# Hi-FT/ERD

Measured on AMD Instinct MI355X. Metric: images/sec GFL-R50 40+40 incre step @1333x800, higher is better.
Workload: dtype f32; 1 GPU; gfl_r50_fpn first_40_incre_last_40 ERD (BASELINE configs[1]), 1333x800 padded to 800x1344, fp32, procedural weights; batch_per_gpu=4, global_batch=4, parallelism=dp1

## Files before the change

### erd_amd/csrc/conv_mfma.hip

```cpp
#include <algorithm>
#include <type_traits>
#include "erd_common.h"
#include <stdlib.h>
#ifndef ERD_SGB
#define ERD_SGB 0
#endif

namespace {

typedef float f32x16 __attribute__((ext_vector_type(16)));
typedef __bf16 bf16x8 __attribute__((ext_vector_type(8)));
typedef __bf16 bf16x2v __attribute__((ext_vector_type(2)));
typedef float f32x2v __attribute__((ext_vector_type(2)));

__device__ __forceinline__ float pack_bf16(float a, float b) {
    const f32x2v v = {a, b};
    return __builtin_bit_cast(float, __builtin_convertvector(v, bf16x2v));
}

constexpr int NTHREADS = 256;

#ifdef ERD_IGEMM_TRACE
__device__ unsigned long long g_igemm_trace[1024 * 8];
#define IG_T0(v) const unsigned long long v = __builtin_amdgcn_s_memtime()
#define IG_ACC(slot, v) if (threadIdx.x == 0 && blockIdx.x < 1024) g_igemm_trace[blockIdx.x * 8 + slot] += __builtin_amdgcn_s_memtime() - v
#define IG_SET(slot, val) if (threadIdx.x == 0 && blockIdx.x < 1024) g_igemm_trace[blockIdx.x * 8 + slot] = (val)
#else
#define IG_T0(v)
#define IG_ACC(slot, v)
#define IG_SET(slot, val)
#endif

struct RowInfo {
    int in_off;
    int ih0, iw0;
    int out_off;
};

__device__ __forceinline__ int swz(int row, int chunk) { return chunk ^ ((row >> 1) & 7); }

typedef unsigned int u32x4 __attribute__((ext_vector_type(4)));
constexpr unsigned OOB = 0x7fffffffu;

__device__ __forceinline__ float4 buf_load16(__amdgpu_buffer_rsrc_t r, unsigned byte_off) {
    const u32x4 v = __builtin_amdgcn_raw_buffer_load_b128(r, byte_off, 0, 0);
    return make_float4(__uint_as_float(v.x), __uint_as_float(v.y), __uint_as_float(v.z), __uint_as_float(v.w));
}

typedef int i32x4 __attribute__((ext_vector_type(4)));
__device__ __forceinline__ i32x4 rsrc_words(const void* ptr, int bytes) {
    const unsigned long long a = (unsigned long long)ptr;
    i32x4 r;
    r.x = __builtin_amdgcn_readfirstlane((int)(unsigned)a);
    r.y = __builtin_amdgcn_readfirstlane((int)((a >> 32) & 0xffffu));
    r.z = __builtin_amdgcn_readfirstlane(bytes);
    r.w = 0x00020000;
    return r;
}
__device__ __forceinline__ void glds16(const i32x4 rs, unsigned lds_byte, unsigned voff) {
    asm volatile("s_mov_b32 m0, %0\n\ts_nop 0\n\tbuffer_load_dwordx4 %1, %2, 0 offen lds" ::"s"(lds_byte), "v"(voff), "s"(rs) : "memory");
}
__device__ __forceinline__ void glds_wait_all() { asm volatile("s_waitcnt vmcnt(0)" ::: "memory"); }

struct SkWs {
    int* cnt;
    float* slabs;
    int xcd_order;
    int whole_tiles;
};

int xcd_order_enabled() {
    static const int v = getenv("ERD_XCD") ? atoi(getenv("ERD_XCD")) : 1;
    return v;
}

template <int BM, int BN, int WAVES_M, int WAVES_N, int BKT, int MINW, bool BF = false, bool ST = false, bool AB = false,
          bool OB = false, bool X3 = false, bool RES = false, bool MSK = false,
          bool GL = false>
__global__ __launch_bounds__(WAVES_M * WAVES_N * 64, MINW) void conv_igemm_kernel(const erd_conv_desc p, const int total_tiles,
                                                                     const SkWs ws) {
    constexpr int NT = WAVES_M * WAVES_N * 64;
    constexpr int FM = BM / (WAVES_M * 32);
    constexpr int FN = BN / (WAVES_N * 32);
    constexpr int CH = BKT / 4;
    constexpr int RPP = NT / CH;
    constexpr int AJ = BM / RPP;
    constexpr int BJ = BN / RPP;
    constexpr int KPC = BF ? 8 : 4;
    constexpr int BK = CH * KPC;
    constexpr bool SGB = ERD_SGB;
    static_assert(WAVES_M * WAVES_N == 4 || (WAVES_M * WAVES_N == 8 && BF && !X3), "4 waves (8: bf16 matrix cores only)");
    static_assert(BF || (!AB && !OB), "bf16 storage only with the bf16 matrix cores");
    static_assert(!X3 || (!BF && BKT == 32 && WAVES_N == 1 && FM == 1), "f32x3: fp32 maps, 32-channel slices, 4 x 1 waves");
    static_assert(!GL || X3, "LDS-DMA staging: the three-limb kernel (both operands are stored in LDS exactly as they lie in memory)");
    constexpr unsigned ABYTES = AB ? 2u : 4u;
    constexpr int CHB = X3 ? 4 : CH;
    constexpr int NPL = X3 ? 3 : 1;
    constexpr int RPPB = NT / CHB;
    constexpr int BJX = BN / RPPB;

    extern __shared__ __attribute__((aligned(16))) char smem[];
    float4* As = reinterpret_cast<float4*>(smem);
    float4* Bs = As + 2 * BM * CH;
    constexpr int OPER_BYTES = 2 * (BM * CH + NPL * BN * CHB) * 16;
    constexpr int STAGE_BYTES = 64 * (BN + 4) * 4 + NT * 16;
    constexpr int REGION = OPER_BYTES > STAGE_BYTES ? OPER_BYTES : STAGE_BYTES;
    constexpr int WSTAGE_BYTES = 32 * (BN + 4) * 4;
    constexpr int ROWS_EPI_OFF = X3 ? ((4 * WSTAGE_BYTES + 255) / 256 * 256) : REGION;
    static_assert(!X3 || ROWS_EPI_OFF + BM * (int)sizeof(RowInfo) + 64 + 4 * (BN / 4) * 16 <= OPER_BYTES,
                  "f32x3: row table + column-sum scratch do not fit behind the staging blocks");
    RowInfo* rows = reinterpret_cast<RowInfo*>(smem + (X3 ? 0 : REGION));
    RowInfo* rows_epi = reinterpret_cast<RowInfo*>(smem + ROWS_EPI_OFF);
    int* bcast = reinterpret_cast<int*>(reinterpret_cast<RowInfo*>(smem + ROWS_EPI_OFF) + BM);

    const int tid = threadIdx.x;
    const int ntn = (p.Cout + BN - 1) / BN;
    const int Cin = p.Cin;
    const int cpt = (Cin + BK - 1) / BK;
    const int nkt = p.ntaps * cpt;
    const float* __restrict__ w = p.w;

    const long long U = (long long)total_tiles * nkt;
    const int G = gridDim.x;
    int wg = blockIdx.x;
    if (ws.xcd_order) {
        const int q = G >> 3, r = G & 7, xcd = blockIdx.x & 7, idx = blockIdx.x >> 3;
        wg = (xcd < r ? xcd * (q + 1) : r * (q + 1) + (xcd - r) * q) + idx;
    }
    const long long u_begin = ws.whole_tiles ? ((long long)total_tiles * wg / G) * nkt : (U * wg) / G;
    const long long u_end = ws.whole_tiles ? ((long long)total_tiles * (wg + 1) / G) * nkt : (U * (wg + 1)) / G;

    const int chunk = tid % CH;
    const int r0 = tid / CH;
    auto swzc = [](int row, int c) { return CH == 8 ? (c ^ ((row >> 1) & 7)) : (c ^ ((row >> 2) & 3)); };
    const int wave = tid >> 6, lane = tid & 63;
    const int chunk_l = GL ? (chunk ^ ((r0 >> 1) & 7)) : chunk;
    const int wave_s = __builtin_amdgcn_readfirstlane(wave);
    const int wm = wave / WAVES_N, wn = wave % WAVES_N;
    const int li = lane & 31, h = lane >> 5;

    IG_T0(t_kernel);
    IG_SET(0, t_kernel);
    for (int q_ = 1; q_ < 8; ++q_) { IG_SET(q_, 0ull); }
    for (long long u = u_begin; u < u_end;) {
        IG_T0(t_pro);
        const int tt = (int)(u / nkt);
        const int ks = (int)(u - (long long)tt * nkt);
        int ke = (int)min((long long)nkt, ks + (u_end - u));
        u += ke - ks;
        const int nt = tt % ntn;
        int mt = tt / ntn;

        int s = 0;
#pragma unroll 1
        for (; s < p.nseg - 1; ++s) {
            const int M = p.seg[s].N * p.seg[s].GH * p.seg[s].GW;
            const int tiles = (M + BM - 1) / BM;
            if (mt < tiles) break;
            mt -= tiles;
        }
        const erd_conv_seg& sg = p.seg[s];
        const int IH = sg.IH, IW = sg.IW;
        const float* __restrict__ in = sg.in;
        const int tap_lo = (ST && sg.ntaps) ? sg.tap0 : 0, nt_s = (ST && sg.ntaps) ? sg.ntaps : p.ntaps;
        const int oy_s = (ST && sg.ntaps) ? sg.oy : p.oy, ox_s = (ST && sg.ntaps) ? sg.ox : p.ox;
        const int nkt_t = ST ? nt_s * cpt : nkt;
        if (ST) {
            ke = min(ke, nkt_t);
            if (ks >= ke) continue;
        }

        __syncthreads();
        auto fill_rows = [&](RowInfo* dst) {
            if (tid < BM) {
                const int GHW = sg.GH * sg.GW;
                const int M = sg.N * GHW;
                const int m = mt * BM + tid;
                RowInfo ri;
                if (m < M) {
                    const int n = m / GHW;
                    const int rem = m - n * GHW;
                    const int a = rem / sg.GW;
                    const int b = rem - a * sg.GW;
                    ri.in_off = (int)(n * sg.in_nstride);
                    ri.ih0 = a * p.in_stride;
                    ri.iw0 = b * p.in_stride;
                    ri.out_off = (int)(n * sg.out_nstride) +
                                 ((a * p.out_stride + oy_s) * sg.OW + (b * p.out_stride + ox_s)) * p.Cout;
                } else {
                    ri.in_off = 0;
                    ri.ih0 = -(1 << 28);
                    ri.iw0 = -(1 << 28);
                    ri.out_off = -1;
                }
                dst[tid] = ri;
            }
        };
        if constexpr (!GL) {
            fill_rows(rows);
            __syncthreads();
        }

        unsigned a_base[AJ], a_mask[AJ];
#pragma unroll
        for (int j = 0; j < AJ; ++j) {
            RowInfo ri;
            if constexpr (GL) {
                const int GHW = sg.GH * sg.GW;
                const int m = mt * BM + r0 + RPP * j;
                if (m < sg.N * GHW) {
                    const int n = m / GHW;
                    const int rem = m - n * GHW;
                    const int a = rem / sg.GW;
                    ri.in_off = (int)(n * sg.in_nstride);
                    ri.ih0 = a * p.in_stride;
                    ri.iw0 = (rem - a * sg.GW) * p.in_stride;
                } else {
                    ri.in_off = 0;
                    ri.ih0 = -(1 << 28);
                    ri.iw0 = -(1 << 28);
                }
            } else {
                ri = rows[r0 + RPP * j];
            }
            a_base[j] = (unsigned)(ri.in_off + (ri.ih0 * IW + ri.iw0) * Cin + chunk_l * KPC) * ABYTES;
            unsigned m = 0;
            for (int t = 0; t < nt_s; ++t) {
                const int ih = ri.ih0 + p.dy[tap_lo + t], iw = ri.iw0 + p.dx[tap_lo + t];
                m |= ((unsigned)ih < (unsigned)IH && (unsigned)iw < (unsigned)IW) ? (1u << t) : 0u;
            }
            a_mask[j] = m;
        }
        const int n0 = nt * BN;
        unsigned b_base[X3 ? 1 : BJ];
        unsigned bx_base[X3 ? BJX : 1];
        const int chunkb = tid % CHB, rb0 = tid / CHB;
        const int chunkb_l = GL ? (chunkb ^ ((rb0 >> 2) & 3)) : chunkb;
        if constexpr (X3) {
#pragma unroll
            for (int j = 0; j < BJX; ++j) {
                const int co = n0 + rb0 + RPPB * j;
                bx_base[j] = co < p.Cout ? (unsigned)(co * p.wrow + chunkb_l * 8) * 2u : OOB;
            }
        } else {
#pragma unroll
            for (int j = 0; j < BJ; ++j) {
                const int co = n0 + r0 + RPP * j;
                b_base[j] = co < p.Cout ? (unsigned)(co * p.wrow + chunk * KPC) * (BF ? 2u : 4u) : OOB;
            }
        }
        const __amdgpu_buffer_rsrc_t rs_in = __builtin_amdgcn_make_buffer_rsrc(
            const_cast<float*>(in), 0, (int)((long long)sg.N * sg.in_nstride * ABYTES), 0x00020000);
        const unsigned plane_b = (unsigned)((long long)p.Cout * p.wrow * 2);
        const __amdgpu_buffer_rsrc_t rs_w = __builtin_amdgcn_make_buffer_rsrc(
            X3 ? const_cast<void*>(p.w_x3) : (BF ? const_cast<void*>(p.w_bf16) : (void*)const_cast<float*>(w)), 0,
            (int)((long long)p.Cout * p.wrow * (X3 ? 6 : (BF ? 2 : 4))), 0x00020000);
        if constexpr (X3 && !GL) __syncthreads();

        constexpr bool PD2 = BF && MINW <= 2;
        constexpr int NSET = PD2 ? 2 : 1;
        constexpr int NBL = X3 ? 3 * BJX : BJ;
        float4 ra[GL ? 1 : NSET][GL ? 1 : AJ], rb[GL ? 1 : NSET][GL ? 1 : NBL];
        float4 ra1[NSET][(BF && !AB) ? AJ : 1];
        bool cokb = false;
        int tap = ks / cpt, cc = ks - tap * cpt;
        int adelta = 0, bdelta = 0, ctap = 0;
        bool cok = false, cok1 = false;
        auto slice_begin = [&]() {
            const int cb = cc * BK;
            ctap = tap;
            adelta = ((p.dy[tap_lo + tap] * IW + p.dx[tap_lo + tap]) * Cin + cb) * (int)ABYTES;
            bdelta = (p.wk[tap_lo + tap] + cb) * ((BF || X3) ? 2 : 4);
            cok = cb + chunk_l * KPC < Cin;
            cokb = X3 && cb + chunkb_l * 8 < Cin;
            cok1 = BF && !AB && cb + chunk * KPC + 4 < Cin;
            if (++cc == cpt) { cc = 0; ++tap; }
        };
        typedef __attribute__((address_space(3))) void* lds_ptr_t;
        const unsigned lds0 = (unsigned)(size_t)(lds_ptr_t)smem;
        const i32x4 rw_in = GL ? rsrc_words(in, (int)((long long)sg.N * sg.in_nstride * ABYTES)) : i32x4{0, 0, 0, 0};
        const i32x4 rw_w = GL ? rsrc_words(p.w_x3, (int)((long long)p.Cout * p.wrow * 6)) : i32x4{0, 0, 0, 0};
        auto glds_a = [&](int j, const int buf) {
            const bool ok = cok && ((a_mask[j] >> ctap) & 1u);
            glds16(rw_in, lds0 + (unsigned)(((buf * BM + RPP * j + 8 * wave_s) * CH) * 16), ok ? a_base[j] + (unsigned)adelta : OOB);
        };
        auto glds_b = [&](int j, const int buf) {
            const int pl = j / BJX, jj = j - pl * BJX;
            glds16(rw_w, lds0 + (unsigned)((2 * BM * CH + (buf * 3 + pl) * BN * CHB + (RPPB * jj + 16 * wave_s) * CHB) * 16),
                   cokb ? bx_base[X3 ? jj : 0] + (unsigned)bdelta + (unsigned)pl * plane_b : OOB);
        };
        auto load_a = [&](int j, const int set) {
            const bool ok = cok && ((a_mask[j] >> ctap) & 1u);
            ra[set][j] = buf_load16(rs_in, ok ? a_base[j] + (unsigned)adelta : OOB);
            if (BF && !AB) ra1[set][j] = buf_load16(rs_in, (ok && cok1) ? a_base[j] + (unsigned)adelta + 16u : OOB);
        };
        auto load_b = [&](int j, const int set) {
            if constexpr (X3) {
                const int pl = j / BJX, jj = j - pl * BJX;
                rb[set][j] = buf_load16(rs_w, cokb ? bx_base[jj] + (unsigned)bdelta + (unsigned)pl * plane_b : OOB);
            } else {
                rb[set][j] = buf_load16(rs_w, cok ? b_base[X3 ? 0 : j] + (unsigned)bdelta : OOB);
            }
        };
        auto store_lds = [&](int buf, const int set) {
#pragma unroll
            for (int j = 0; j < AJ; ++j) {
                const int row = r0 + RPP * j;
                if (BF && !AB)
                    As[buf * BM * CH + row * CH + swzc(row, chunk)] =
                        make_float4(pack_bf16(ra[set][j].x, ra[set][j].y), pack_bf16(ra[set][j].z, ra[set][j].w),
                                    pack_bf16(ra1[set][(BF && !AB) ? j : 0].x, ra1[set][(BF && !AB) ? j : 0].y),
                                    pack_bf16(ra1[set][(BF && !AB) ? j : 0].z, ra1[set][(BF && !AB) ? j : 0].w));
                else
                    As[buf * BM * CH + row * CH + swzc(row, chunk)] = ra[set][j];
            }
            if constexpr (X3) {
#pragma unroll
                for (int j = 0; j < 3 * BJX; ++j) {
                    const int pl = j / BJX, row = rb0 + RPPB * (j - pl * BJX);
                    Bs[(buf * 3 + pl) * BN * CHB + row * CHB + (chunkb ^ ((row >> 2) & 3))] = rb[set][j];
                }
            } else {
#pragma unroll
                for (int j = 0; j < BJ; ++j) {
                    const int row = r0 + RPP * j;
                    Bs[buf * BN * CH + row * CH + swzc(row, chunk)] = rb[set][X3 ? 0 : j];
                }
            }
        };

        f32x16 acc[FM][FN];
#pragma unroll
        for (int i = 0; i < FM; ++i)
#pragma unroll
            for (int j = 0; j < FN; ++j)
#pragma unroll
                for (int r = 0; r < 16; ++r) acc[i][j][r] = 0.f;

        slice_begin();
        if constexpr (GL) {
#pragma unroll
            for (int j = 0; j < NBL; ++j) glds_b(j, 0);
#pragma unroll
            for (int j = 0; j < AJ; ++j) glds_a(j, 0);
        } else {
#pragma unroll
        for (int j = 0; j < AJ; ++j) load_a(j, 0);
#pragma unroll
        for (int j = 0; j < NBL; ++j) load_b(j, 0);
        }
        if (PD2 && ks + 1 < ke) {
            slice_begin();
#pragma unroll
            for (int j = 0; j < AJ; ++j) load_a(j, NSET - 1);
#pragma unroll
            for (int j = 0; j < NBL; ++j) load_b(j, NSET - 1);
        }
        if constexpr (GL) glds_wait_all(); else store_lds(0, 0);
        __syncthreads();

        IG_ACC(2, t_pro);
        IG_T0(t_loop);
        constexpr int KSTEPS = X3 ? 2 : CH / 2;
        constexpr int APS = (AJ + KSTEPS - 1) / KSTEPS, BPS = (NBL + KSTEPS - 1) / KSTEPS;
        auto k_slice_x3 = [&](const int kt, const int par) {
            const int buf = par;
            const bool more = kt + 1 < ke;
            if (more) slice_begin();
            const float4* Ab = As + buf * BM * CH;
            const float4* Bb = Bs + buf * 3 * BN * CHB;
            const int arow = wm * 32 + li;
            typedef unsigned int u4v __attribute__((ext_vector_type(4)));
            auto limb = [&](const float (&v)[8], u4v& P) {
#pragma unroll
                for (int e = 0; e < 4; ++e) P[e] = erd::pack2_bf16(v[2 * e], v[2 * e + 1]);
                return __builtin_bit_cast(bf16x8, P);
            };
            auto rest = [&](const float (&v)[8], const u4v& P, float (&r)[8]) {
#pragma unroll
                for (int e = 0; e < 4; ++e) {
                    r[2 * e] = erd::scalar_op(v[2 * e] - erd::bf16_lo(P[e]));
                    r[2 * e + 1] = erd::scalar_op(v[2 * e + 1] - erd::bf16_hi(P[e]));
                }
            };
            auto read_a = [&](int kk, float (&x)[8]) {
                const int ca = 4 * kk + 2 * h;
                const float4 x0 = Ab[arow * CH + swzc(arow, ca)], x1 = Ab[arow * CH + swzc(arow, ca + 1)];
                x[0] = x0.x; x[1] = x0.y; x[2] = x0.z; x[3] = x0.w; x[4] = x1.x; x[5] = x1.y; x[6] = x1.z; x[7] = x1.w;
            };
            float4 wb[FN][3];
            auto read_b = [&](int kk, const int pl) {
                const int cbk = 2 * kk + h;
#pragma unroll
                for (int j = 0; j < FN; ++j) {
                    const int row = j * 32 + li;
                    wb[j][pl] = Bb[pl * BN * CHB + row * CHB + (cbk ^ ((row >> 2) & 3))];
                }
            };
#ifdef ERD_X3_NOMFMA
#define ERD_X3(AV, PL)                                                                                              \
            _Pragma("unroll") for (int j = 0; j < FN; ++j) acc[0][j][PL] += wb[j][PL].x * __builtin_bit_cast(float4, AV).x;
#else
#define ERD_X3(AV, PL)                                                                                              \
            _Pragma("unroll") for (int j = 0; j < FN; ++j)                                                          \
                acc[0][j] = __builtin_amdgcn_mfma_f32_32x32x16_bf16(AV, __builtin_bit_cast(bf16x8, wb[j][PL]), acc[0][j], 0, 0, 0);
#endif
            float x[8], xn[8];
            read_a(0, x);
            read_b(0, 2);
            read_b(0, 1);
            read_b(0, 0);
#pragma unroll
            for (int kk = 0; kk < 2; ++kk) {
                if (kk == 0) read_a(1, xn);
#ifndef ERD_X3_NOLOAD
                if (more) {
#pragma unroll
                    for (int q = 0; q < APS; ++q)
                        if (kk * APS + q < AJ) { if constexpr (GL) glds_a(kk * APS + q, buf ^ 1); else load_a(kk * APS + q, 0); }
#pragma unroll
                    for (int q = 0; q < BPS; ++q)
                        if (kk * BPS + q < NBL) { if constexpr (GL) glds_b(kk * BPS + q, buf ^ 1); else load_b(kk * BPS + q, 0); }
                }
#endif
                u4v ph, pm, pl;
                const bf16x8 ah = limb(x, ph);
                ERD_X3(ah, 2)
#ifndef ERD_X3_NOBREAD
                if (kk == 0) read_b(1, 2);
#endif
                ERD_X3(ah, 1)
                ERD_X3(ah, 0)
                float r1[8], r2[8];
#ifdef ERD_X3_NOVALU
                const bf16x8 am = ah, al = ah;
                (void)r1; (void)r2;
#else
                rest(x, ph, r1);
                const bf16x8 am = limb(r1, pm);
#endif
                ERD_X3(am, 1)
#ifndef ERD_X3_NOBREAD
                if (kk == 0) read_b(1, 1);
#endif
                ERD_X3(am, 0)
#ifndef ERD_X3_NOVALU
                rest(r1, pm, r2);
                const bf16x8 al = limb(r2, pl);
#endif
                ERD_X3(al, 0)
#ifdef ERD_X3_NINE
                ERD_X3(am, 2)
                ERD_X3(al, 1)
                ERD_X3(al, 2)
#endif
                if (kk == 0) {
#ifndef ERD_X3_NOBREAD
                    read_b(1, 0);
#endif
#pragma unroll
                    for (int e = 0; e < 8; ++e) x[e] = xn[e];
                }
            }
#undef ERD_X3
#ifndef ERD_X3_NOSYNC
            if constexpr (GL) glds_wait_all(); else { if (more) store_lds(buf ^ 1, 0); }
            __syncthreads();
#endif
        };
        auto k_slice = [&](const int kt, const int par) {
            const int buf = par;
            const bool more = kt + 1 < ke;
            const bool fetch = PD2 ? kt + 2 < ke : more;
            const int fset = PD2 ? par : 0;
            if (fetch) slice_begin();
            const float4* Ab = As + buf * BM * CH;
            const float4* Bb = Bs + buf * BN * CH;
            float4 fa[2][FM], fb[2][FN];
            auto read_frags = [&](int kk, int slot) {
                const int c = 2 * kk + h;
#pragma unroll
                for (int i = 0; i < FM; ++i) {
                    const int row = (wm * FM + i) * 32 + li;
                    fa[slot][i] = Ab[row * CH + swzc(row, c)];
                }
#pragma unroll
                for (int j = 0; j < FN; ++j) {
                    const int row = (wn * FN + j) * 32 + li;
                    fb[slot][j] = Bb[row * CH + swzc(row, c)];
                }
            };
            read_frags(0, 0);
#pragma unroll
            for (int kk = 0; kk < KSTEPS; ++kk) {
                const int cur = kk & 1;
#ifndef ERD_IG_NOFRAG
                if (kk + 1 < KSTEPS) read_frags(kk + 1, cur ^ 1);
#endif
#ifdef ERD_IG_NOLOAD
                if (false) {
#else
                if (fetch) {
#endif
#pragma unroll
                    for (int q = 0; q < APS; ++q)
                        if (kk * APS + q < AJ) load_a(kk * APS + q, fset);
#pragma unroll
                    for (int q = 0; q < BPS; ++q)
                        if (kk * BPS + q < BJ) load_b(kk * BPS + q, fset);
                }
#pragma unroll
                for (int i = 0; i < FM; ++i)
#pragma unroll
                    for (int j = 0; j < FN; ++j) {
                        if (BF) {
#ifdef ERD_IG_NOMFMA
                            acc[i][j][kk] += fa[cur][i].x * fb[cur][j].y;
                            continue;
#endif
                            acc[i][j] = __builtin_amdgcn_mfma_f32_32x32x16_bf16(
                                __builtin_bit_cast(bf16x8, fa[cur][i]), __builtin_bit_cast(bf16x8, fb[cur][j]),
                                acc[i][j], 0, 0, 0);
                            continue;
                        }
                        acc[i][j] = __builtin_amdgcn_mfma_f32_32x32x2f32(fa[cur][i].x, fb[cur][j].x, acc[i][j], 0, 0, 0);
                        acc[i][j] = __builtin_amdgcn_mfma_f32_32x32x2f32(fa[cur][i].y, fb[cur][j].y, acc[i][j], 0, 0, 0);
                        acc[i][j] = __builtin_amdgcn_mfma_f32_32x32x2f32(fa[cur][i].z, fb[cur][j].z, acc[i][j], 0, 0, 0);
                        acc[i][j] = __builtin_amdgcn_mfma_f32_32x32x2f32(fa[cur][i].w, fb[cur][j].w, acc[i][j], 0, 0, 0);
                    }
                if (SGB) {
                    __builtin_amdgcn_sched_group_barrier(0x100, FM + FN, 0);
                    __builtin_amdgcn_sched_group_barrier(0x20, APS + BPS, 0);
                    __builtin_amdgcn_sched_group_barrier(0x8, FM * FN * 4, 0);
                }
            }
#ifndef ERD_IG_NOSYNC
            if (more) store_lds(buf ^ 1, PD2 ? (par ^ 1) : 0);
            __syncthreads();
#endif
        };
        if constexpr (X3) {
            for (int kt = ks; kt < ke; ++kt) k_slice_x3(kt, (kt - ks) & 1);
        } else if constexpr (PD2) {
            for (int kt = ks; kt < ke; kt += 2) {
                k_slice(kt, 0);
                if (kt + 1 < ke) k_slice(kt + 1, 1);
            }
        } else {
            for (int kt = ks; kt < ke; ++kt) k_slice(kt, (kt - ks) & 1);
        }

        IG_ACC(3, t_loop);
        IG_SET(6, g_igemm_trace[blockIdx.x * 8 + 6] + (unsigned long long)(ke - ks));
        IG_T0(t_fix);
        if (ks != 0 || ke != nkt_t) {
            const long long t0 = (long long)tt * nkt;
            const int first_b = (int)(((t0 + 1) * G - 1) / U);
            const int last_b = (int)(((t0 + nkt) * G - 1) / U);
            const int ncontrib = last_b - first_b + 1;
            const int my_slot = (tt == (int)(u_begin / nkt)) ? 0 : 1;
            const __amdgpu_buffer_rsrc_t rs_slab = __builtin_amdgcn_make_buffer_rsrc(
                ws.slabs, 0, (int)std::min<size_t>((size_t)2 * G * BM * BN * 4, 0x7fffffffu), 0x00020000);
            const unsigned slab_off = (unsigned)((size_t)(2 * wg + my_slot) * (BM * BN) * 4) + (unsigned)tid * 16u;
#pragma unroll
            for (int i = 0; i < FM; ++i)
#pragma unroll
                for (int j = 0; j < FN; ++j)
#pragma unroll
                    for (int g = 0; g < 4; ++g) {
                        u32x4 v;
                        v.x = __float_as_uint(acc[i][j][4 * g]); v.y = __float_as_uint(acc[i][j][4 * g + 1]);
                        v.z = __float_as_uint(acc[i][j][4 * g + 2]); v.w = __float_as_uint(acc[i][j][4 * g + 3]);
                        __builtin_amdgcn_raw_buffer_store_b128(v, rs_slab, slab_off + (unsigned)(((i * FN + j) * 4 + g) * NT * 16), 0, 16 );
                    }
            asm volatile("s_waitcnt vmcnt(0)" ::: "memory");
            __syncthreads();
            if (tid == 0) bcast[0] = __hip_atomic_fetch_add(ws.cnt + tt, 1, __ATOMIC_RELAXED, __HIP_MEMORY_SCOPE_AGENT);
            __syncthreads();
            if (bcast[0] != ncontrib - 1) { IG_ACC(4, t_fix); IG_SET(1, __builtin_amdgcn_s_memtime()); continue; }
            const bool pair = ncontrib == 2;
            if (!pair) {
#pragma unroll
                for (int i = 0; i < FM; ++i)
#pragma unroll
                    for (int j = 0; j < FN; ++j)
#pragma unroll
                        for (int r = 0; r < 16; ++r) acc[i][j][r] = 0.f;
            }
            for (int c = 0; c < ncontrib; ++c) {
                const int bb = first_b + c;
                if (pair && bb == wg) continue;
                const int bfirst_tile = (int)(((U * bb) / G) / nkt);
                const unsigned so = (unsigned)((size_t)(2 * bb + (tt == bfirst_tile ? 0 : 1)) * (BM * BN) * 4) + (unsigned)tid * 16u;
#pragma unroll
                for (int i = 0; i < FM; ++i)
#pragma unroll
                    for (int j = 0; j < FN; ++j)
#pragma unroll
                        for (int g = 0; g < 4; ++g) {
                            const u32x4 v = __builtin_amdgcn_raw_buffer_load_b128(
                                rs_slab, so + (unsigned)(((i * FN + j) * 4 + g) * NT * 16), 0, 16 );
                            acc[i][j][4 * g] += __uint_as_float(v.x); acc[i][j][4 * g + 1] += __uint_as_float(v.y);
                            acc[i][j][4 * g + 2] += __uint_as_float(v.z); acc[i][j][4 * g + 3] += __uint_as_float(v.w);
                        }
            }
            if (tid == 0) ws.cnt[tt] = 0;
        }

        IG_ACC(4, t_fix);
        IG_T0(t_epi);
        if constexpr (X3) fill_rows(rows_epi);
        using OutT = typename std::conditional<OB, erd::bf16s, float>::type;
        OutT* __restrict__ out = reinterpret_cast<OutT*>(sg.out);
        const OutT* res = reinterpret_cast<const OutT*>(sg.res);
        const OutT* msk = reinterpret_cast<const OutT*>(sg.mask);
        const float alpha = sg.alpha ? *sg.alpha : 1.f;
        const bool has_alpha = sg.alpha != nullptr;
        float* stage = reinterpret_cast<float*>(smem);
        constexpr int SLD = BN + 4;
        constexpr int C4N = BN / 4;
        constexpr int RPS = NT / C4N;
        if constexpr (X3) {
            {
                __syncthreads();
                float* wst = reinterpret_cast<float*>(smem + wave * WSTAGE_BYTES);
                constexpr int RPW = 64 / C4N, NIT = 32 / RPW;
                const int c4 = lane % C4N, rsub = lane / C4N;
                const int co = n0 + c4 * 4;
                const bool cvalid = co < p.Cout;
                const int out_bytes = erd::uniform_int((int)((long long)sg.N * sg.out_nstride * 4));
                const __amdgpu_buffer_rsrc_t rs_out = __builtin_amdgcn_make_buffer_rsrc(erd::uniform_ptr(sg.out), 0, out_bytes, 0x00020000);
                const __amdgpu_buffer_rsrc_t rs_res = __builtin_amdgcn_make_buffer_rsrc(
                    erd::uniform_ptr(const_cast<float*>(sg.res ? sg.res : sg.out)), 0, erd::uniform_int(sg.res ? out_bytes : 0), 0x00020000);
                const __amdgpu_buffer_rsrc_t rs_msk = __builtin_amdgcn_make_buffer_rsrc(
                    erd::uniform_ptr(const_cast<float*>(sg.mask ? sg.mask : sg.out)), 0, erd::uniform_int(sg.mask ? out_bytes : 0), 0x00020000);
                const bool no_msk = sg.mask == nullptr;
                auto row_off = [&](int q) -> unsigned {
                    const int oo = rows_epi[wave * 32 + q * RPW + rsub].out_off;
                    return (oo < 0 || !cvalid) ? OOB : (unsigned)(oo + co) * 4u;
                };
                constexpr int NP = (RES && MSK) ? NIT / 4 : NIT / 2, NPQ = NP < 4 ? NP : 4;
                float4 pr[RES ? NP : 1], pm[MSK ? NP : 1];
                if constexpr (RES) {
#pragma unroll
                    for (int q = 0; q < NPQ; ++q) pr[q] = buf_load16(rs_res, row_off(q));
                } else if constexpr (MSK) {
#pragma unroll
                    for (int q = 0; q < NPQ; ++q) pm[q] = buf_load16(rs_msk, row_off(q));
                }
#pragma unroll
                for (int j = 0; j < FN; ++j)
#pragma unroll
                    for (int r = 0; r < 16; ++r) wst[((r & 3) + 8 * (r >> 2) + 4 * h) * SLD + j * 32 + li] = acc[0][j][r];
                if constexpr (RES) {
#pragma unroll
                    for (int q = NPQ; q < NP; ++q) pr[q] = buf_load16(rs_res, row_off(q));
                }
                if constexpr (MSK) {
#pragma unroll
                    for (int q = RES ? 0 : NPQ; q < NP; ++q) pm[q] = buf_load16(rs_msk, row_off(q));
                }
                float4 sc = make_float4(1.f, 1.f, 1.f, 1.f), sh = make_float4(0.f, 0.f, 0.f, 0.f);
                if (cvalid && p.scale) sc = *reinterpret_cast<const float4*>(p.scale + co);
                if (cvalid && p.shift) sh = *reinterpret_cast<const float4*>(p.shift + co);
                __builtin_amdgcn_wave_barrier();
                asm volatile("s_waitcnt lgkmcnt(0)" ::: "memory");
                float4 csum = make_float4(0.f, 0.f, 0.f, 0.f);
#pragma unroll
                for (int ph = 0; ph < NIT / NP; ++ph) {
                    if (ph > 0) {
                        if constexpr (RES) {
#pragma unroll
                            for (int q = 0; q < NP; ++q) pr[q] = buf_load16(rs_res, row_off(ph * NP + q));
                        }
                        if constexpr (MSK) {
#pragma unroll
                            for (int q = 0; q < NP; ++q) pm[q] = buf_load16(rs_msk, row_off(ph * NP + q));
                        }
                    }
#pragma unroll
                    for (int qq = 0; qq < NP; ++qq) {
                        const int q = ph * NP + qq;
                        const int rr = q * RPW + rsub;
                        float4 v = *reinterpret_cast<const float4*>(wst + rr * SLD + c4 * 4);
                        v.x = v.x * sc.x + sh.x; v.y = v.y * sc.y + sh.y; v.z = v.z * sc.z + sh.z; v.w = v.w * sc.w + sh.w;
                        if (has_alpha) { v.x *= alpha; v.y *= alpha; v.z *= alpha; v.w *= alpha; }
                        if constexpr (RES) { const float4 rv = pr[qq]; v.x += rv.x; v.y += rv.y; v.z += rv.z; v.w += rv.w; }
                        if (p.relu) { v.x = fmaxf(v.x, 0.f); v.y = fmaxf(v.y, 0.f); v.z = fmaxf(v.z, 0.f); v.w = fmaxf(v.w, 0.f); }
                        if constexpr (MSK) {
                            const float4 mv = pm[qq];
                            v.x = (mv.x > 0.f || no_msk) ? v.x : 0.f; v.y = (mv.y > 0.f || no_msk) ? v.y : 0.f;
                            v.z = (mv.z > 0.f || no_msk) ? v.z : 0.f; v.w = (mv.w > 0.f || no_msk) ? v.w : 0.f;
                        }
                        const unsigned o = row_off(q);
                        __builtin_amdgcn_raw_buffer_store_b128(__builtin_bit_cast(u32x4, v), rs_out, o, 0, 0);
                        if (o != OOB) { csum.x += v.x; csum.y += v.y; csum.z += v.z; csum.w += v.w; }
                    }
                }
                if (p.colsum) {
#pragma unroll
                    for (int o = C4N; o < 64; o <<= 1) {
                        csum.x += __shfl_xor(csum.x, o, 64); csum.y += __shfl_xor(csum.y, o, 64);
                        csum.z += __shfl_xor(csum.z, o, 64); csum.w += __shfl_xor(csum.w, o, 64);
                    }
                    float4* red = reinterpret_cast<float4*>(smem + ROWS_EPI_OFF + BM * sizeof(RowInfo) + 64);
                    if (lane < C4N) red[wave * C4N + lane] = cvalid ? csum : make_float4(0.f, 0.f, 0.f, 0.f);
                    __syncthreads();
                    if (tid < C4N && n0 + tid * 4 < p.Cout) {
                        float4 t = red[tid];
                        for (int q = 1; q < 4; ++q) { const float4 v = red[q * C4N + tid]; t.x += v.x; t.y += v.y; t.z += v.z; t.w += v.w; }
                        float* cs = p.colsum + (p.colsum_copies > 1 ? (int64_t)(blockIdx.x & (p.colsum_copies - 1)) * p.Cout : 0);
                        const int cc0 = n0 + tid * 4;
                        atomicAdd(cs + cc0 + 0, t.x); atomicAdd(cs + cc0 + 1, t.y); atomicAdd(cs + cc0 + 2, t.z); atomicAdd(cs + cc0 + 3, t.w);
                    }
                }
            }
        }
#pragma unroll
        for (int half = 0; half < (X3 ? 0 : WAVES_M); ++half) {
            __syncthreads();
            constexpr int NPF = (FM * 32) / RPS;
            constexpr bool PREFETCH = MINW <= 3;
            float4 pf[PREFETCH ? NPF : 1];
            const OutT* pf_src = res ? res : msk;
            if (PREFETCH && pf_src && (p.Cout & 3) == 0 && n0 + (tid % C4N) * 4 < p.Cout) {
#pragma unroll
                for (int q = 0; q < NPF; ++q) {
                    const int oo = rows_epi[half * FM * 32 + tid / C4N + q * RPS].out_off;
                    if (oo >= 0) pf[PREFETCH ? q : 0] = erd::ld4(pf_src + oo + n0 + (tid % C4N) * 4);
                }
            }
            if (wm == half) {
#pragma unroll
                for (int i = 0; i < FM; ++i)
#pragma unroll
                    for (int j = 0; j < FN; ++j)
#pragma unroll
                        for (int r = 0; r < 16; ++r) {
                            const int row = i * 32 + (r & 3) + 8 * (r >> 2) + 4 * h;
                            stage[row * SLD + (wn * FN + j) * 32 + li] = acc[i][j][r];
                        }
            }
            __syncthreads();
            const int c4 = tid % C4N;
            const int co = n0 + c4 * 4;
            float4 csum_keep = make_float4(0.f, 0.f, 0.f, 0.f);
            if (co < p.Cout && (p.Cout & 3) != 0) {
                float csum[4] = {0.f, 0.f, 0.f, 0.f};
                for (int rr = tid / C4N; rr < FM * 32; rr += RPS) {
                    const int oo = rows_epi[half * FM * 32 + rr].out_off;
                    if (oo < 0) continue;
#pragma unroll
                    for (int e = 0; e < 4; ++e) {
                        if (co + e >= p.Cout) break;
                        float x = stage[rr * SLD + c4 * 4 + e];
                        x = x * (p.scale ? p.scale[co + e] : 1.f) + (p.shift ? p.shift[co + e] : 0.f);
                        if (has_alpha) x *= alpha;
                        if (res) x += erd::ld1(res + oo + co + e);
                        if (p.relu) x = fmaxf(x, 0.f);
                        if (msk) x = erd::ld1(msk + oo + co + e) > 0.f ? x : 0.f;
                        erd::st1(out + oo + co + e, x);
                        csum[e] += x;
                    }
                }
                if (p.colsum) csum_keep = make_float4(csum[0], csum[1], csum[2], csum[3]);
            } else if (co < p.Cout) {
                float4 sc = make_float4(1.f, 1.f, 1.f, 1.f), sh = make_float4(0.f, 0.f, 0.f, 0.f);
                if (p.scale) sc = *reinterpret_cast<const float4*>(p.scale + co);
                if (p.shift) sh = *reinterpret_cast<const float4*>(p.shift + co);
                float4 csum = make_float4(0.f, 0.f, 0.f, 0.f);
#pragma unroll
                for (int q = 0; q < NPF; ++q) {
                    const int rr = tid / C4N + q * RPS;
                    const int oo = rows_epi[half * FM * 32 + rr].out_off;
                    if (oo < 0) continue;
                    float4 v = *reinterpret_cast<const float4*>(stage + rr * SLD + c4 * 4);
                    v.x = v.x * sc.x + sh.x; v.y = v.y * sc.y + sh.y; v.z = v.z * sc.z + sh.z; v.w = v.w * sc.w + sh.w;
                    if (has_alpha) { v.x *= alpha; v.y *= alpha; v.z *= alpha; v.w *= alpha; }
                    if (res) {
                        const float4 rv = PREFETCH ? pf[PREFETCH ? q : 0] : erd::ld4(res + oo + co);
                        v.x += rv.x; v.y += rv.y; v.z += rv.z; v.w += rv.w;
                    }
                    if (p.relu) { v.x = fmaxf(v.x, 0.f); v.y = fmaxf(v.y, 0.f); v.z = fmaxf(v.z, 0.f); v.w = fmaxf(v.w, 0.f); }
                    if (msk) {
                        const float4 mv = (PREFETCH && !res) ? pf[PREFETCH ? q : 0] : erd::ld4(msk + oo + co);
                        v.x = mv.x > 0.f ? v.x : 0.f; v.y = mv.y > 0.f ? v.y : 0.f;
                        v.z = mv.z > 0.f ? v.z : 0.f; v.w = mv.w > 0.f ? v.w : 0.f;
                    }
                    erd::st4(out + oo + co, v);
                    csum.x += v.x; csum.y += v.y; csum.z += v.z; csum.w += v.w;
                }
                if (p.colsum) csum_keep = csum;
            }
            if (p.colsum) {
                float4* red = reinterpret_cast<float4*>(stage + 64 * SLD);
                __syncthreads();
                red[tid] = (co < p.Cout) ? csum_keep : make_float4(0.f, 0.f, 0.f, 0.f);
                __syncthreads();
                if (tid < C4N && co < p.Cout) {
                    float4 t = red[tid];
                    for (int q = 1; q < RPS; ++q) {
                        const float4 v = red[q * C4N + tid];
                        t.x += v.x; t.y += v.y; t.z += v.z; t.w += v.w;
                    }
                    float* cs = p.colsum + (p.colsum_copies > 1 ? (int64_t)(blockIdx.x & (p.colsum_copies - 1)) * p.Cout : 0);
                    atomicAdd(cs + co + 0, t.x);
                    if (co + 1 < p.Cout) atomicAdd(cs + co + 1, t.y);
                    if (co + 2 < p.Cout) atomicAdd(cs + co + 2, t.z);
                    if (co + 3 < p.Cout) atomicAdd(cs + co + 3, t.w);
                }
            }
        }
        IG_ACC(5, t_epi);
        IG_SET(1, __builtin_amdgcn_s_memtime());
    }
}

template <int BM, int BN, int BKW, int MINW>
__global__ __launch_bounds__(NTHREADS, MINW) void conv_wgrad_kernel(const erd_wgrad_desc p, const int xcd_order) {
    constexpr int BK = BKW;
    constexpr int FM = BM / 64, FN = BN / 64;
    constexpr int AC = BM / 4, BC = BN / 4;
    constexpr int AJ = (BK * AC) / NTHREADS, BJ = (BK * BC) / NTHREADS;
    constexpr int AR = NTHREADS / AC, BR = NTHREADS / BC;
    extern __shared__ __attribute__((aligned(16))) char smem[];
    float* As = reinterpret_cast<float*>(smem);
    float* Bs = As + 2 * BK * BM;
    int2* offs = reinterpret_cast<int2*>(Bs + 2 * BK * BN);

    const int tid = threadIdx.x;
    const int nci = (p.Cin + BN - 1) / BN;
    int wg = blockIdx.x;
    if (xcd_order) {
        const int G = gridDim.x, q = G >> 3, r = G & 7, xcd = blockIdx.x & 7, idx = blockIdx.x >> 3;
        wg = (xcd < r ? xcd * (q + 1) : r * (q + 1) + (xcd - r) * q) + idx;
    }
    const int nxb = nci * p.ntaps, nyb = (p.Cout + BM - 1) / BM;
    const int bx = wg % nxb, by = (wg / nxb) % nyb, bz = wg / (nxb * nyb);
    const int tap = bx / nci;
    const int ci0 = (bx % nci) * BN;
    const int co0 = by * BM;
    int P = 0;
    for (int l = 0; l < p.nseg; ++l) P += p.seg[l].N * p.seg[l].GH * p.seg[l].GW;
    const int nkt_total = (P + BK - 1) / BK;
    const int per = (nkt_total + p.nsplit - 1) / p.nsplit;
    const int kt_begin = bz * per;
    const int kt_end = min(nkt_total, kt_begin + per);
    const int dyt = p.dy[tap], dxt = p.dx[tap];
    const float* __restrict__ x = p.x;
    const float* __restrict__ dz = p.dz;

    const int achunk = tid % AC, ar0 = tid / AC;
    const int bchunk = tid % BC, br0 = tid / BC;
    const bool a_cok = co0 + achunk * 4 < p.Cout;
    const bool b_cok = ci0 + bchunk * 4 < p.Cin;
    const int a_col = co0 + achunk * 4, b_col = ci0 + bchunk * 4;

    auto compute_offsets = [&](int kt, int slot) {
        if (tid < BK) {
            int pp = kt * BK + tid;
            int2 o = make_int2(-1, -1);
            if (pp < P && kt < kt_end) {
                int l = 0;
#pragma unroll 1
                for (; l < p.nseg - 1; ++l) {
                    const int pl = p.seg[l].N * p.seg[l].GH * p.seg[l].GW;
                    if (pp < pl) break;
                    pp -= pl;
                }
                const erd_wgrad_seg& g = p.seg[l];
                const int GHW = g.GH * g.GW;
                const int n = pp / GHW;
                const int rem = pp - n * GHW;
                const int a = rem / g.GW;
                const int b = rem - a * g.GW;
                o.x = (int)(g.dz_off + n * g.dz_nstride) +
                      ((a * p.out_stride + p.oy) * g.OW + (b * p.out_stride + p.ox)) * p.Cout;
                const int ih = a * p.in_stride + dyt, iw = b * p.in_stride + dxt;
                if ((unsigned)ih < (unsigned)g.IH && (unsigned)iw < (unsigned)g.IW)
                    o.y = (int)(g.x_off + n * g.x_nstride) + (ih * g.IW + iw) * p.Cin;
            }
            offs[slot * BK + tid] = o;
        }
    };

    const __amdgpu_buffer_rsrc_t rs_dz = __builtin_amdgcn_make_buffer_rsrc(
        const_cast<float*>(dz), 0, (int)(p.dz_elems * 4), 0x00020000);
    const __amdgpu_buffer_rsrc_t rs_x = __builtin_amdgcn_make_buffer_rsrc(
        const_cast<float*>(x), 0, (int)(p.x_elems * 4), 0x00020000);
    float4 ra[AJ], rb[BJ];
    auto load_global = [&](int slot) {
#pragma unroll
        for (int j = 0; j < AJ; ++j) {
            const int o = offs[slot * BK + ar0 + AR * j].x;
            ra[j] = buf_load16(rs_dz, (o >= 0 && a_cok) ? (unsigned)(o + a_col) * 4u : OOB);
        }
#pragma unroll
        for (int j = 0; j < BJ; ++j) {
            const int o = offs[slot * BK + br0 + BR * j].y;
            rb[j] = buf_load16(rs_x, (o >= 0 && b_cok) ? (unsigned)(o + b_col) * 4u : OOB);
        }
    };
    auto store_lds = [&](int buf) {
#pragma unroll
        for (int j = 0; j < AJ; ++j)
            *reinterpret_cast<float4*>(As + (buf * BK + ar0 + AR * j) * BM + achunk * 4) = ra[j];
#pragma unroll
        for (int j = 0; j < BJ; ++j)
            *reinterpret_cast<float4*>(Bs + (buf * BK + br0 + BR * j) * BN + bchunk * 4) = rb[j];
    };

    const int wave = tid >> 6, lane = tid & 63;
    const int wm = wave >> 1, wn = wave & 1;
    const int li = lane & 31, h = lane >> 5;
    f32x16 acc[FM][FN];
#pragma unroll
    for (int i = 0; i < FM; ++i)
#pragma unroll
        for (int j = 0; j < FN; ++j)
#pragma unroll
            for (int r = 0; r < 16; ++r) acc[i][j][r] = 0.f;

    if (kt_begin < kt_end) {
        compute_offsets(kt_begin, 0);
        __syncthreads();
        load_global(0);
        compute_offsets(kt_begin + 1, 1);
        store_lds(0);
        __syncthreads();
        for (int kt = kt_begin; kt < kt_end; ++kt) {
            const int buf = (kt - kt_begin) & 1;
            const bool more = kt + 1 < kt_end;
            if (more) load_global(buf ^ 1);
            compute_offsets(kt + 2, buf);
            const float* Ab = As + buf * BK * BM;
            const float* Bb = Bs + buf * BK * BN;
#pragma unroll
            for (int ks = 0; ks < BK / 2; ++ks) {
                const int k = 2 * ks + h;
                float fa[FM], fb[FN];
#pragma unroll
                for (int i = 0; i < FM; ++i) fa[i] = Ab[k * BM + (wm * FM + i) * 32 + li];
#pragma unroll
                for (int j = 0; j < FN; ++j) fb[j] = Bb[k * BN + (wn * FN + j) * 32 + li];
#pragma unroll
                for (int i = 0; i < FM; ++i)
#pragma unroll
                    for (int j = 0; j < FN; ++j)
                        acc[i][j] = __builtin_amdgcn_mfma_f32_32x32x2f32(fa[i], fb[j], acc[i][j], 0, 0, 0);
            }
            if (more) store_lds(buf ^ 1);
            __syncthreads();
        }
    }
    float* __restrict__ part = p.part + (int64_t)bz * p.Cout * p.ntaps * p.Cin;
#pragma unroll
    for (int j = 0; j < FN; ++j) {
        const int ci = ci0 + (wn * FN + j) * 32 + li;
        if (ci >= p.Cin) continue;
#pragma unroll
        for (int i = 0; i < FM; ++i)
#pragma unroll
            for (int r = 0; r < 16; ++r) {
                const int co = co0 + (wm * FM + i) * 32 + (r & 3) + 8 * (r >> 2) + 4 * h;
                if (co < p.Cout) part[((int64_t)co * p.ntaps + tap) * p.Cin + ci] = acc[i][j][r];
            }
    }
}
// ... 1151 lines not shown
```

Baseline: 120.6 images/sec.

## Interleave global-to-LDS loads between MFMA instructions in x3 bf16 conv path

In the GL/X3 implicit-GEMM path, the next slice's buffer_load...lds requests are no longer issued in a burst before each k-step. They are spread into the gaps after selected MFMA instructions of the first k16 step. Inline-asm ties to the accumulators pin each load's position in the instruction schedule, and the loop is peeled so the last slice issues no prefetch. The prologue also issues the B loads before decoding the row addresses, to overlap address math with memory traffic. Adds finer-grained trace instrumentation under a debug macro. The risk is schedule constraints that hurt MFMA issue or add register pressure.

Result: faster. 122.4 images/sec, median of 6 (+1.5%).

```diff
diff --git a/erd_amd/csrc/conv_mfma.hip b/erd_amd/csrc/conv_mfma.hip
--- a/erd_amd/csrc/conv_mfma.hip
+++ b/erd_amd/csrc/conv_mfma.hip
@@ -21,14 +21,28 @@
 constexpr int NTHREADS = 256;
 
 #ifdef ERD_IGEMM_TRACE
-__device__ unsigned long long g_igemm_trace[1024 * 8];
+constexpr int IG_NS = 32;
+__device__ unsigned long long g_igemm_trace[1024 * IG_NS];
 #define IG_T0(v) const unsigned long long v = __builtin_amdgcn_s_memtime()
-#define IG_ACC(slot, v) if (threadIdx.x == 0 && blockIdx.x < 1024) g_igemm_trace[blockIdx.x * 8 + slot] += __builtin_amdgcn_s_memtime() - v
-#define IG_SET(slot, val) if (threadIdx.x == 0 && blockIdx.x < 1024) g_igemm_trace[blockIdx.x * 8 + slot] = (val)
+#define IG_ACC(slot, v) if (threadIdx.x == 0 && blockIdx.x < 1024) g_igemm_trace[blockIdx.x * IG_NS + slot] += __builtin_amdgcn_s_memtime() - v
+#define IG_SET(slot, val) if (threadIdx.x == 0 && blockIdx.x < 1024) g_igemm_trace[blockIdx.x * IG_NS + slot] = (val)
+#define IG_LAPS_DECL unsigned ig_lap[IG_NS] = {}; unsigned ig_prev = 0
+#define IG_MARK() do { __builtin_amdgcn_sched_barrier(0); ig_prev = (unsigned)__builtin_amdgcn_s_memtime(); __builtin_amdgcn_sched_barrier(0); } while (0)
+#define IG_LAP(slot) do { __builtin_amdgcn_sched_barrier(0); const unsigned t_ = (unsigned)__builtin_amdgcn_s_memtime();     \
+                          ig_lap[slot] += t_ - ig_prev; ig_prev = t_; __builtin_amdgcn_sched_barrier(0); } while (0)
+#define IG_G_FIRST int ig_g = 0
+#define IG_G_NEXT ++ig_g
+#define IG_LAPS_STORE() for (int q_ = 7; q_ < IG_NS; ++q_) { IG_SET(q_, (unsigned long long)ig_lap[q_]); }
 #else
 #define IG_T0(v)
 #define IG_ACC(slot, v)
 #define IG_SET(slot, val)
+#define IG_LAPS_DECL
+#define IG_MARK()
+#define IG_LAP(slot)
+#define IG_G_FIRST
+#define IG_G_NEXT
+#define IG_LAPS_STORE()
 #endif
 
 struct RowInfo {
@@ -48,6 +62,7 @@
 }
 
 typedef int i32x4 __attribute__((ext_vector_type(4)));
+template <bool B> struct bool_c { static constexpr bool value = B; };
 __device__ __forceinline__ i32x4 rsrc_words(const void* ptr, int bytes) {
     const unsigned long long a = (unsigned long long)ptr;
     i32x4 r;
@@ -57,8 +72,27 @@
     r.w = 0x00020000;
     return r;
 }
+#pragma clang diagnostic push
+#pragma clang diagnostic ignored "-Winline-asm"
+template <bool FRESH = false>
 __device__ __forceinline__ void glds16(const i32x4 rs, unsigned lds_byte, unsigned voff) {
-    asm volatile("s_mov_b32 m0, %0\n\ts_nop 0\n\tbuffer_load_dwordx4 %1, %2, 0 offen lds" ::"s"(lds_byte), "v"(voff), "s"(rs) : "memory");
+    if constexpr (FRESH)
+        asm volatile("s_nop 4\n\ts_mov_b32 m0, %0\n\ts_nop 0\n\tbuffer_load_dwordx4 %1, %2, 0 offen lds" ::"s"(lds_byte), "v"(voff), "s"(rs)
+                     : "memory", "m0");
+    else
+        asm volatile("s_mov_b32 m0, %0\n\ts_nop 0\n\tbuffer_load_dwordx4 %1, %2, 0 offen lds" ::"s"(lds_byte), "v"(voff), "s"(rs) : "memory", "m0");
+}
+typedef float f32x16_t __attribute__((ext_vector_type(16)));
+__device__ __forceinline__ void glds16(const i32x4 rs, unsigned lds_byte, unsigned voff, f32x16_t& after, f32x16_t& before) {
+    asm volatile("s_mov_b32 m0, %2\n\ts_nop 0\n\tbuffer_load_dwordx4 %3, %4, 0 offen lds"
+                 : "+v"(after), "+v"(before)
+                 : "s"(lds_byte), "v"(voff), "s"(rs)
+                 : "memory", "m0");
+}
+#pragma clang diagnostic pop
+template <bool FRESH, typename... T>
+__device__ __forceinline__ void glds16_sel(bool_c<FRESH>, const i32x4 rs, unsigned lds_byte, unsigned voff, T&... tie) {
+    if constexpr (sizeof...(T) == 0) glds16<FRESH>(rs, lds_byte, voff); else glds16(rs, lds_byte, voff, tie...);
 }
 __device__ __forceinline__ void glds_wait_all() { asm volatile("s_waitcnt vmcnt(0)" ::: "memory"); }
 
@@ -142,6 +176,7 @@
     IG_T0(t_kernel);
     IG_SET(0, t_kernel);
     for (int q_ = 1; q_ < 8; ++q_) { IG_SET(q_, 0ull); }
+    IG_LAPS_DECL;
     for (long long u = u_begin; u < u_end;) {
         IG_T0(t_pro);
         const int tt = (int)(u / nkt);
@@ -202,35 +237,37 @@
         }
 
         unsigned a_base[AJ], a_mask[AJ];
-#pragma unroll
-        for (int j = 0; j < AJ; ++j) {
-            RowInfo ri;
-            if constexpr (GL) {
-                const int GHW = sg.GH * sg.GW;
-                const int m = mt * BM + r0 + RPP * j;
-                if (m < sg.N * GHW) {
-                    const int n = m / GHW;
-                    const int rem = m - n * GHW;
-                    const int a = rem / sg.GW;
-                    ri.in_off = (int)(n * sg.in_nstride);
-                    ri.ih0 = a * p.in_stride;
-                    ri.iw0 = (rem - a * sg.GW) * p.in_stride;
-                } else {
-                    ri.in_off = 0;
-                    ri.ih0 = -(1 << 28);
-                    ri.iw0 = -(1 << 28);
-                }
-            } else {
-                ri = rows[r0 + RPP * j];
-            }
-            a_base[j] = (unsigned)(ri.in_off + (ri.ih0 * IW + ri.iw0) * Cin + chunk_l * KPC) * ABYTES;
-            unsigned m = 0;
-            for (int t = 0; t < nt_s; ++t) {
-                const int ih = ri.ih0 + p.dy[tap_lo + t], iw = ri.iw0 + p.dx[tap_lo + t];
-                m |= ((unsigned)ih < (unsigned)IH && (unsigned)iw < (unsigned)IW) ? (1u << t) : 0u;
-            }
-            a_mask[j] = m;
-        }
+#define ERD_DECODE_ROWS                                                                                                                            \
+        _Pragma("unroll")                                                                                                                          \
+        for (int j = 0; j < AJ; ++j) {                                                                                                             \
+            RowInfo ri;                                                                                                                            \
+            if constexpr (GL) {         \
+                const int GHW = sg.GH * sg.GW;                                                                                                     \
+                const int m = mt * BM + r0 + RPP * j;                                                                                              \
+                if (m < sg.N * GHW) {                                                                                                              \
+                    const int n = m / GHW;                                                                                                         \
+                    const int rem = m - n * GHW;                                                                                                   \
+                    const int a = rem / sg.GW;                                                                                                     \
+                    ri.in_off = (int)(n * sg.in_nstride);                                                                                          \
+                    ri.ih0 = a * p.in_stride;                                                                                                      \
+                    ri.iw0 = (rem - a * sg.GW) * p.in_stride;                                                                                      \
+                } else {                                                                                                                           \
+                    ri.in_off = 0;                                                                                                                 \
+                    ri.ih0 = -(1 << 28);                                                                                                           \
+                    ri.iw0 = -(1 << 28);                                                                                                           \
+                }                                                                                                                                  \
+            } else {                                                                                                                               \
+                ri = rows[r0 + RPP * j];                                                                                                           \
+            }                                                                                                                                      \
+            a_base[j] = (unsigned)(ri.in_off + (ri.ih0 * IW + ri.iw0) * Cin + chunk_l * KPC) * ABYTES;                                             \
+            unsigned m = 0;                                                                                                                        \
+            for (int t = 0; t < nt_s; ++t) {                                                                                                       \
+                const int ih = ri.ih0 + p.dy[tap_lo + t], iw = ri.iw0 + p.dx[tap_lo + t];                                                          \
+                m |= ((unsigned)ih < (unsigned)IH && (unsigned)iw < (unsigned)IW) ? (1u << t) : 0u;                                                \
+            }                                                                                                                                      \
+            a_mask[j] = m;                                                                                                                         \
+        }
+        if constexpr (!GL) { ERD_DECODE_ROWS }
         const int n0 = nt * BN;
         unsigned b_base[X3 ? 1 : BJ];
         unsigned bx_base[X3 ? BJX : 1];
@@ -280,14 +317,14 @@
         const unsigned lds0 = (unsigned)(size_t)(lds_ptr_t)smem;
         const i32x4 rw_in = GL ? rsrc_words(in, (int)((long long)sg.N * sg.in_nstride * ABYTES)) : i32x4{0, 0, 0, 0};
         const i32x4 rw_w = GL ? rsrc_words(p.w_x3, (int)((long long)p.Cout * p.wrow * 6)) : i32x4{0, 0, 0, 0};
-        auto glds_a = [&](int j, const int buf) {
+        auto glds_a = [&](int j, const int buf, auto&... tie) {
             const bool ok = cok && ((a_mask[j] >> ctap) & 1u);
-            glds16(rw_in, lds0 + (unsigned)(((buf * BM + RPP * j + 8 * wave_s) * CH) * 16), ok ? a_base[j] + (unsigned)adelta : OOB);
+            glds16(rw_in, lds0 + (unsigned)(((buf * BM + RPP * j + 8 * wave_s) * CH) * 16), ok ? a_base[j] + (unsigned)adelta : OOB, tie...);
         };
-        auto glds_b = [&](int j, const int buf) {
+        auto glds_b = [&](int j, const int buf, auto fresh, auto&... tie) {
             const int pl = j / BJX, jj = j - pl * BJX;
-            glds16(rw_w, lds0 + (unsigned)((2 * BM * CH + (buf * 3 + pl) * BN * CHB + (RPPB * jj + 16 * wave_s) * CHB) * 16),
-                   cokb ? bx_base[X3 ? jj : 0] + (unsigned)bdelta + (unsigned)pl * plane_b : OOB);
+            glds16_sel(fresh, rw_w, lds0 + (unsigned)((2 * BM * CH + (buf * 3 + pl) * BN * CHB + (RPPB * jj + 16 * wave_s) * CHB) * 16),
+                   cokb ? bx_base[X3 ? jj : 0] + (unsigned)bdelta + (unsigned)pl * plane_b : OOB, tie...);
         };
         auto load_a = [&](int j, const int set) {
             const bool ok = cok && ((a_mask[j] >> ctap) & 1u);
@@ -337,12 +374,22 @@
 #pragma unroll
                 for (int r = 0; r < 16; ++r) acc[i][j][r] = 0.f;
 
-        slice_begin();
+#ifdef ERD_GLP_BURST
+        constexpr bool SPLIT = false;
+#else
+        constexpr bool SPLIT = GL;
+#endif
+        if constexpr (!GL) slice_begin();
         if constexpr (GL) {
-#pragma unroll
-            for (int j = 0; j < NBL; ++j) glds_b(j, 0);
+            slice_begin();
+            glds_b(0, 0, bool_c<true>{});
+#pragma unroll
+            for (int j = 1; j < NBL; ++j) glds_b(j, 0, bool_c<false>{});
+            { ERD_DECODE_ROWS }
 #pragma unroll
             for (int j = 0; j < AJ; ++j) glds_a(j, 0);
+            glds_wait_all();
+#undef ERD_DECODE_ROWS
         } else {
 #pragma unroll
         for (int j = 0; j < AJ; ++j) load_a(j, 0);
@@ -356,17 +403,36 @@
 #pragma unroll
             for (int j = 0; j < NBL; ++j) load_b(j, NSET - 1);
         }
-        if constexpr (GL) glds_wait_all(); else store_lds(0, 0);
+        if constexpr (!GL) store_lds(0, 0);
         __syncthreads();
 
         IG_ACC(2, t_pro);
         IG_T0(t_loop);
         constexpr int KSTEPS = X3 ? 2 : CH / 2;
         constexpr int APS = (AJ + KSTEPS - 1) / KSTEPS, BPS = (NBL + KSTEPS - 1) / KSTEPS;
-        auto k_slice_x3 = [&](const int kt, const int par) {
+#ifndef ERD_GLP_SLOTS
+#define ERD_GLP_SLOTS 0x5
+#endif
+#ifndef ERD_GLP_AFIRST
+#define ERD_GLP_AFIRST 0
+#endif
+        constexpr int NP = AJ + NBL;
+        constexpr unsigned GLP_SLOTS = FN >= 4 ? (unsigned)(ERD_GLP_SLOTS) : 0x3u;
+        constexpr int GLP_NSLOT = 6 * __builtin_popcount(GLP_SLOTS & ((1u << FN) - 1u));
+        static_assert(!SPLIT || NP <= GLP_NSLOT, "a slice's requests do not fit the MFMA gaps of its first k16 step");
+        auto k_slice_x3 = [&](const int kt, const int par, auto more_c) {
+            constexpr bool MORE = decltype(more_c)::value;
             const int buf = par;
-            const bool more = kt + 1 < ke;
+            const bool more = SPLIT ? MORE : kt + 1 < ke;
             if (more) slice_begin();
+            IG_MARK();
+            int np = 0;
+            auto request = [&](const int i, const int j) {
+                const int ia = ERD_GLP_AFIRST ? i : i - NBL, ib = ERD_GLP_AFIRST ? i - AJ : i;
+                f32x16 &t0 = acc[0][j], &t1 = acc[0][(j + 1) % FN];
+                if (ia >= 0 && ia < AJ) glds_a(ia, buf ^ 1, t0, t1);
+                if (ib >= 0 && ib < NBL) glds_b(ib, buf ^ 1, bool_c<false>{}, t0, t1);
+            };
             const float4* Ab = As + buf * BM * CH;
             const float4* Bb = Bs + buf * 3 * BN * CHB;
             const int arow = wm * 32 + li;
@@ -402,8 +468,11 @@
             _Pragma("unroll") for (int j = 0; j < FN; ++j) acc[0][j][PL] += wb[j][PL].x * __builtin_bit_cast(float4, AV).x;
 #else
 #define ERD_X3(AV, PL)                                                                                              \
-            _Pragma("unroll") for (int j = 0; j < FN; ++j)                                                          \
-                acc[0][j] = __builtin_amdgcn_mfma_f32_32x32x16_bf16(AV, __builtin_bit_cast(bf16x8, wb[j][PL]), acc[0][j], 0, 0, 0);
+            _Pragma("unroll") for (int j = 0; j < FN; ++j) {                                                        \
+                acc[0][j] = __builtin_amdgcn_mfma_f32_32x32x16_bf16(AV, __builtin_bit_cast(bf16x8, wb[j][PL]), acc[0][j], 0, 0, 0); \
+                if constexpr (SPLIT && MORE) { if (((GLP_SLOTS >> j) & 1) && np < NP) request(np++, j); }   \
+            }                                                                                                       \
+            IG_LAP(16 + 6 * kk + ig_g); IG_G_NEXT;
 #endif
             float x[8], xn[8];
             read_a(0, x);
@@ -413,16 +482,21 @@
 #pragma unroll
             for (int kk = 0; kk < 2; ++kk) {
                 if (kk == 0) read_a(1, xn);
+                IG_LAP(8 + kk);
 #ifndef ERD_X3_NOLOAD
+                if constexpr (!SPLIT) {
                 if (more) {
 #pragma unroll
                     for (int q = 0; q < APS; ++q)
                         if (kk * APS + q < AJ) { if constexpr (GL) glds_a(kk * APS + q, buf ^ 1); else load_a(kk * APS + q, 0); }
 #pragma unroll
                     for (int q = 0; q < BPS; ++q)
-                        if (kk * BPS + q < NBL) { if constexpr (GL) glds_b(kk * BPS + q, buf ^ 1); else load_b(kk * BPS + q, 0); }
+                        if (kk * BPS + q < NBL) { if constexpr (GL) glds_b(kk * BPS + q, buf ^ 1, bool_c<false>{}); else load_b(kk * BPS + q, 0); }
+                }
                 }
 #endif
+                IG_LAP(10 + kk);
+                IG_G_FIRST;
                 u4v ph, pm, pl;
                 const bf16x8 ah = limb(x, ph);
                 ERD_X3(ah, 2)
@@ -464,8 +538,11 @@
             }
 #undef ERD_X3
 #ifndef ERD_X3_NOSYNC
+            IG_LAP(12);
             if constexpr (GL) glds_wait_all(); else { if (more) store_lds(buf ^ 1, 0); }
+            IG_LAP(13);
             __syncthreads();
+            IG_LAP(7);
 #endif
         };
         auto k_slice = [&](const int kt, const int par) {
@@ -539,8 +616,11 @@
             __syncthreads();
 #endif
         };
-        if constexpr (X3) {
-            for (int kt = ks; kt < ke; ++kt) k_slice_x3(kt, (kt - ks) & 1);
+        if constexpr (X3 && SPLIT) {
+            for (int kt = ks; kt + 1 < ke; ++kt) k_slice_x3(kt, (kt - ks) & 1, bool_c<true>{});
+            k_slice_x3(ke - 1, (ke - 1 - ks) & 1, bool_c<false>{});
+        } else if constexpr (X3) {
+            for (int kt = ks; kt < ke; ++kt) k_slice_x3(kt, (kt - ks) & 1, bool_c<false>{});
         } else if constexpr (PD2) {
             for (int kt = ks; kt < ke; kt += 2) {
                 k_slice(kt, 0);
@@ -551,7 +631,7 @@
         }
 
         IG_ACC(3, t_loop);
-        IG_SET(6, g_igemm_trace[blockIdx.x * 8 + 6] + (unsigned long long)(ke - ks));
+        IG_SET(6, g_igemm_trace[blockIdx.x * IG_NS + 6] + (unsigned long long)(ke - ks));
         IG_T0(t_fix);
         if (ks != 0 || ke != nkt_t) {
             const long long t0 = (long long)tt * nkt;
@@ -814,6 +894,7 @@
         IG_ACC(5, t_epi);
         IG_SET(1, __builtin_amdgcn_s_memtime());
     }
+    IG_LAPS_STORE();
 }
 
 template <int BM, int BN, int BKW, int MINW>
```
